# typesense/typesense

Measured on NVIDIA B200. Metric: queries/sec, higher is better.
Workload: dtype u32+f32

## Files before the change

### include/tsgpu.h

```cpp
#ifndef TSGPU_H
#define TSGPU_H
#include <stdint.h>
#include <stddef.h>

#ifdef __cplusplus
extern "C" {
#endif

typedef int tsgpu_status;
enum {
    TSGPU_OK = 0,
    TSGPU_ERR_NO_DEVICE = 1,
    TSGPU_ERR_INVALID = 2,
    TSGPU_ERR_CUDA = 3,
    TSGPU_ERR_CAPACITY = 4
};

#define TSGPU_NO_LIST 0xFFFFFFFFu
#define TSGPU_MAX_FIELDS 8
#define TSGPU_MAX_TOKENS 16
#define TSGPU_MAX_TOPK 1024

typedef struct tsgpu_index tsgpu_index;

// ... 189 lines not shown
typedef struct { uint32_t value_id, count, doc_id, array_pos; } tsgpu_facet_count;
tsgpu_status tsgpu_index_load_facet(tsgpu_index* idx, const tsgpu_facet* f, uint32_t* out_facet);
tsgpu_status tsgpu_facet_counts(tsgpu_index* idx, uint32_t facet, const uint32_t* result_ids, size_t n, uint32_t sample_mod,
                                uint32_t top_n, tsgpu_facet_count* out, uint32_t* out_n, uint32_t* out_distinct);
tsgpu_status tsgpu_facet_counts_last(tsgpu_index* idx, uint32_t facet, uint32_t top_n, tsgpu_facet_count* out, uint32_t* out_n,
                                     uint32_t* out_distinct);
tsgpu_status tsgpu_all_result_ids_last(tsgpu_index* idx, uint32_t q, uint32_t* out_ids, size_t cap, size_t* out_n);

typedef struct {
    float    ms_total;
    float    ms_kernels;
    float    ms_keyword;
    float    ms_knn;
    float    ms_fuse;
    uint64_t launches_total;
    uint64_t kw_driver_ids;
    uint64_t kw_probe_ids;
    uint64_t kw_matches;
    uint64_t knn_dist;
    uint64_t knn_expanded;
    uint64_t h2d_bytes;
    uint64_t d2h_bytes;
    float    ms_kw_search;
    float    ms_kw_merge;
    float    ms_host_plan;
    uint64_t knn_spec_hits;
    uint64_t knn_tier2_walks;
    uint64_t knn_retried;
    uint64_t h2d_total;
    uint64_t d2h_total;
    uint64_t calls_total;
    uint64_t knn_table_probes;
    uint64_t flat_tc_queries;
} tsgpu_stats;
tsgpu_status tsgpu_get_stats(tsgpu_index* idx, tsgpu_stats* out);
tsgpu_status tsgpu_debug_knn_work(tsgpu_index* idx, uint32_t* out, uint32_t cap_queries, uint32_t* out_n);

#ifdef __cplusplus
}
#endif
#endif
```

### typesense_b200/csrc/knn_kernels.cuh

```cuda
#pragma once
#include <cuda_runtime.h>
#include <stdint.h>
#include <float.h>

namespace tsv {

constexpr uint32_t kNone = 0xFFFFFFFFu;
constexpr int kKnnThreads = 128;
constexpr uint32_t kCandSmem = 256;
constexpr uint32_t kVisSmem = 2048;
constexpr uint32_t kVisSmemLimit = 1536;

struct HnswDev {
    uint32_t n_nodes, dim, M, max_level, entry_point, metric;
    const float* vectors;
    const uint32_t* labels;
    const uint8_t* levels;
    const uint32_t* links0;
    const unsigned long long* upper_off;
    const uint32_t* links_up;
    const uint32_t* deleted;
};

struct KnnParams {
    const float* queries;
    uint32_t nq, k, ef;
    const uint32_t* const* q_filter_bitmap;
    const uint32_t* const* q_excl;
    const uint32_t* q_n_excl;
    const uint8_t* q_skip;
    const uint32_t* q_order;
    uint32_t n_order;
    const uint32_t* n_order_dev;
    float* out_dist;
    uint32_t* out_labels;
    uint32_t* out_n;
    uint32_t* vis2;
    uint32_t vis2_slots;
    unsigned long long* cand;
    uint32_t cand_cap;
    uint32_t* counter;
    unsigned long long* stats;
    uint32_t* retry_n;
    uint32_t* retry_list;
    uint32_t vis_cache;
    uint32_t walk_prefetch;
    uint32_t* q_work;
};

__device__ __forceinline__ uint32_t ord_f32(float f) {
    const uint32_t u = __float_as_uint(f);
    return (u & 0x80000000u) ? ~u : (u | 0x80000000u);
}
__device__ __forceinline__ float unord_f32(uint32_t o) {
    const uint32_t u = (o & 0x80000000u) ? (o & 0x7FFFFFFFu) : ~o;
    return __uint_as_float(u);
}

template <int NCH>
struct QReg { float4 v[NCH > 0 ? NCH : 1]; };

__device__ __forceinline__ float warp_tree(float a0, float a1, float a2, float a3) {
    float t = __fadd_rn(__fadd_rn(a0, a1), __fadd_rn(a2, a3));
#pragma unroll
    for(int off = 16; off >= 1; off >>= 1) t = __fadd_rn(t, __shfl_xor_sync(0xffffffffu, t, off));
    return t;
}

template <int NCH>
__device__ __forceinline__ float dot_one(const QReg<NCH>& q, const float* __restrict__ qs, const float* __restrict__ v,
                                         uint32_t dim, uint32_t lane) {
    float a0 = 0.f, a1 = 0.f, a2 = 0.f, a3 = 0.f;
    if(NCH > 0) {
        float4 x[NCH > 0 ? NCH : 1];
#pragma unroll
        for(int s = 0; s < NCH; s++) x[s] = __ldg(reinterpret_cast<const float4*>(v + s * 128) + lane);
#pragma unroll
        for(int s = 0; s < NCH; s++) {
            a0 = __fmaf_rn(q.v[s].x, x[s].x, a0); a1 = __fmaf_rn(q.v[s].y, x[s].y, a1);
// ... 474 lines not shown
    asm volatile("mbarrier.init.shared::cta.b64 [%0], %1;" :: "r"(bar), "r"(count) : "memory");
}
__device__ __forceinline__ void mbar_expect_tx(uint32_t bar, uint32_t bytes) {
    asm volatile("mbarrier.arrive.expect_tx.shared::cta.b64 _, [%0], %1;" :: "r"(bar), "r"(bytes) : "memory");
}
__device__ __forceinline__ bool mbar_try_wait(uint32_t bar, uint32_t parity) {
    uint32_t ok;
    asm volatile("{\n\t.reg .pred p;\n\tmbarrier.try_wait.parity.shared::cta.b64 p, [%1], %2;\n\tselp.u32 %0, 1, 0, p;\n\t}"
                 : "=r"(ok) : "r"(bar), "r"(parity) : "memory");
    return ok != 0;
}
__device__ __forceinline__ void bulk_g2s(uint32_t dst, const void* src, uint32_t bytes, uint32_t bar) {
    asm volatile("cp.async.bulk.shared::cluster.global.mbarrier::complete_tx::bytes [%0], [%1], %2, [%3];"
                 :: "r"(dst), "l"(src), "r"(bytes), "r"(bar) : "memory");
}

__device__ __forceinline__ bool vis_test_and_set(uint32_t* cache, uint32_t cmask, uint32_t* table, uint32_t mask2, uint32_t node, bool* went_to_table = nullptr) {
    const uint32_t key = node + 1;
    const uint32_t h = vis_hash(node);
    uint32_t* c = cache + (h & cmask);
    if(*c == key) return false;
    if(went_to_table) *went_to_table = true;
    bool fresh = false;
    uint32_t j = (h >> 11) & mask2;
    for(;;) {
        const uint32_t old = atomicCAS(table + j, 0u, key);
        if(old == 0) { fresh = true; break; }
        if(old == key) break;
        j = (j + 1) & mask2;
    }
    *c = key;
    return fresh;
}

#ifndef TSGPU_WALK_MIN_CTAS
#define TSGPU_WALK_MIN_CTAS 5
#endif
template <int NCH, int RS>
__global__ void __launch_bounds__(32 * kWalkWarps, RS == 2 ? 2 * TSGPU_WALK_MIN_CTAS : (RS == 8 ? 2 : TSGPU_WALK_MIN_CTAS))
hnsw_walk_kernel(const __grid_constant__ HnswDev g, const __grid_constant__ KnnParams P) {
    extern __shared__ __align__(128) unsigned char smem_raw[];
    const uint32_t lane = threadIdx.x & 31, warp = threadIdx.x >> 5;
    const uint32_t slot = blockIdx.x * kWalkWarps + warp;
    const uint32_t ef = P.ef > P.k ? P.ef : P.k;
    constexpr uint32_t dim = NCH * 128, row_bytes = dim * 4;
    unsigned long long* bars = reinterpret_cast<unsigned long long*>(smem_raw);
    float* ring = reinterpret_cast<float*>(smem_raw + 128) + (size_t) warp * RS * dim;
    const uint32_t n_cache = P.vis_cache, cmask = n_cache - 1;
    uint32_t* cache = reinterpret_cast<uint32_t*>(smem_raw + 128 + (size_t) kWalkWarps * RS * row_bytes) + (size_t) warp * n_cache;
    const uint32_t bar = smem_u32(bars + warp), ring_s = smem_u32(ring);
    uint32_t parity = 0;
    if(lane == 0) mbar_init(bar, 1);
    asm volatile("fence.mbarrier_init.release.cluster;" ::: "memory");
    __syncwarp();
    uint32_t* vis2 = P.vis2 + (size_t) slot * P.vis2_slots;
    const uint32_t mask2 = P.vis2_slots - 1;
    const uint32_t limit2 = P.vis2_slots - (P.vis2_slots >> 2);
    unsigned long long* const pool0 = P.cand + (size_t) slot * P.cand_cap;
    const uint32_t pool_half = P.cand_cap >> 1;
    const uint32_t L0 = 2 * g.M + 1, LU = g.M + 1;
    const uint32_t n_tickets = P.n_order_dev ? __ldcg(P.n_order_dev) : (P.q_order ? P.n_order : P.nq);
    unsigned long long n_dist_acc = 0, n_exp_acc = 0, n_hit_acc = 0, n_t2_acc = 0, n_tab_acc = 0;
    float* const qs = nullptr;

    for(;;) {
        uint32_t qi = 0;
        if(lane == 0) qi = atomicAdd(P.counter, 1u);
        qi = __shfl_sync(0xffffffffu, qi, 0);
        if(qi >= n_tickets) break;
        if(P.q_order) qi = __ldg(P.q_order + qi);
        if(P.q_skip && P.q_skip[qi]) { if(lane == 0) P.out_n[qi] = 0; continue; }
        const float* qv = P.queries + (size_t) qi * dim;
        QReg<NCH> q;
#pragma unroll
        for(int s = 0; s < NCH; s++) q.v[s] = __ldg(reinterpret_cast<const float4*>(qv + s * 128) + lane);
        const uint32_t* fbm = P.q_filter_bitmap ? P.q_filter_bitmap[qi] : nullptr;
        const uint32_t* excl = P.q_excl ? P.q_excl[qi] : nullptr;
        const uint32_t n_excl = P.q_n_excl ? P.q_n_excl[qi] : 0;
        if(g.n_nodes == 0 || g.entry_point == kNone) { if(lane == 0) P.out_n[qi] = 0; continue; }
        for(uint32_t i = lane; i < n_cache; i += 32) cache[i] = 0;
        const unsigned long long exp0 = n_exp_acc, dist0 = n_dist_acc;

        uint32_t cur = g.entry_point;
        float curdist = 1.0f - dot_one<NCH>(q, qs, g.vectors + (size_t) cur * dim, dim, lane);
        n_dist_acc++;
        for(int level = (int) g.max_level; level > 0; level--) {
            bool changed = true;
            while(changed) {
                changed = false;
                const uint32_t* rec = g.links_up + (g.upper_off[cur] + (unsigned long long) (level - 1)) * LU;
                const uint32_t size = __ldg(rec);
                const uint32_t nb = (lane < size) ? __ldg(rec + 1 + lane) : kNone;
                for(uint32_t i = 0; i < size; i += 2) {
                    const uint32_t c0 = __shfl_sync(0xffffffffu, nb, i);
                    const uint32_t c1 = (i + 1 < size) ? __shfl_sync(0xffffffffu, nb, i + 1) : c0;
                    float d0, d1;
// ... 5 lines not shown
                }
            }
        }

        WArr<kResPerLane> R; warr_clear(R);
        WArr<kBufPerLane> B; warr_clear(B);
        uint32_t n_res = 0, n_b = 0;
        unsigned long long* nearp = pool0;
        unsigned long long* farp = pool0 + pool_half;
        uint32_t n_near = 0, n_far = 0;
        unsigned long long pv = kKeyInf;
        unsigned long long b_last = 0;
        uint32_t n_vis = 0;
        bool overflow = false;
        float lowerBound;
        __syncwarp();
        {
            const bool ok = allowed(g, fbm, excl, n_excl, cur);
            if(ok) {
                const float d = curdist;
                n_dist_acc++;
                lowerBound = d;
                warr_insert(R, res_key(d, cur), lane); n_res = 1;
                warr_insert(B, cand_key(d, cur), lane); n_b = 1; b_last = cand_key(d, cur);
            } else {
                lowerBound = FLT_MAX;
                warr_insert(B, cand_key(FLT_MAX, cur), lane); n_b = 1; b_last = cand_key(FLT_MAX, cur);
            }
            if(lane == 0) vis_test_and_set(cache, cmask, vis2, mask2, cur);
            n_vis = 1;
            __syncwarp();
        }
        uint32_t prev_spec = kNone, prev_nb2 = kNone, prev_size2 = 0;
        for(;;) {
            if(overflow) break;
            if(n_b == 0) {
                if(n_near == 0) {
                    if(n_far == 0) break;
                    unsigned long long* t = nearp; nearp = farp; farp = t;
                    n_near = n_far; n_far = 0; pv = kKeyInf;
                }
                __syncwarp();
                if(n_near > kNearMax) {
                    const uint32_t n = n_near;
                    const unsigned long long sk = nearp[(unsigned long long) lane * n >> 5];
                    uint32_t rank = 0;
#pragma unroll 8
                    for(int o = 0; o < 32; o++) rank += __shfl_sync(0xffffffffu, sk, o) < sk ? 1u : 0u;
                    uint32_t q = (32u * kNearTarget + (n >> 1)) / n;
                    q = q < 1 ? 1 : (q > 16 ? 16 : q);
                    const unsigned long long pivot = __shfl_sync(0xffffffffu, sk, __ffs(__ballot_sync(0xffffffffu, rank == q)) - 1);
                    uint32_t w = 0;
                    const uint32_t lt = (1u << lane) - 1u;
                    for(uint32_t base = 0; base < n; base += 32) {
                        const bool valid = base + lane < n;
                        const unsigned long long k = valid ? nearp[base + lane] : kKeyInf;
                        const uint32_t mb = __ballot_sync(0xffffffffu, valid && k < pivot);
                        const uint32_t ma = __ballot_sync(0xffffffffu, valid && k >= pivot);
                        if(n_far + __popc(ma) > pool_half) { overflow = true; break; }
                        if(valid) {
                            if(k < pivot) nearp[w + __popc(mb & lt)] = k;
                            else farp[n_far + __popc(ma & lt)] = k;
                        }
                        w += __popc(mb); n_far += __popc(ma);
                    }
                    if(overflow) break;
// ... 32 lines not shown
                        C = N;
                    }
                    n_near = n;
                    b_last = warr_get(B, n_b - 1);
                }
                __syncwarp();
            }
            const unsigned long long top = warr_front(B);
            const float cdist = unord_f32((uint32_t) (top >> 32));
            if(cdist > lowerBound && n_res == ef) break;
            const uint32_t cnode = ~(uint32_t) top;
            warr_pop_front(B, lane); n_b--;
            if(n_b == 0) b_last = 0;
            n_exp_acc++;

            const uint32_t* rec = g.links0 + (size_t) cnode * L0;
            const bool reuse = cnode == prev_spec;
            n_hit_acc += reuse ? 1 : 0;
            const uint32_t size = reuse ? prev_size2 : __ldg(rec);
            const uint32_t nb = reuse ? prev_nb2 : ((lane + 1 < L0) ? __ldg(rec + 1 + lane) : kNone);
            uint32_t spec = kNone, nb2 = kNone, size2 = 0;
            if(n_b) spec = ~(uint32_t) warr_front(B);
            if(spec != kNone) {
                const uint32_t* rec2 = g.links0 + (size_t) spec * L0;
                size2 = __ldg(rec2);
                nb2 = (lane + 1 < L0) ? __ldg(rec2 + 1 + lane) : kNone;
            }
            if(n_vis + 32 > limit2) { overflow = true; break; }
            uint32_t fw = 0xffffffffu, dw = 0u;
            if(lane < size && !g.labels) {
                if(fbm) fw = __ldg(fbm + (nb >> 5));
                if(g.deleted) dw = __ldg(g.deleted + (nb >> 5));
            }
            bool to_table = false;
            const bool fresh = (lane < size) && vis_test_and_set(cache, cmask, vis2, mask2, nb, &to_table);
            uint32_t mask = __ballot_sync(0xffffffffu, fresh);
            n_vis += __popc(mask);
            n_tab_acc += __popc(__ballot_sync(0xffffffffu, to_table));
            bool ok_mine = false;
            if(fresh) {
                if(g.labels) ok_mine = allowed(g, fbm, excl, n_excl, nb);
                else ok_mine = ((fw >> (nb & 31)) & 1u) && !((dw >> (nb & 31)) & 1u) && !(n_excl && is_excluded(excl, n_excl, nb));
            }
            const uint32_t ok_mask = __ballot_sync(0xffffffffu, ok_mine);
            n_dist_acc += __popc(mask);
            bool hinted = P.walk_prefetch == 0;
            auto hint_next = [&]() {
                hinted = true;
                if(spec != kNone && lane < size2) {
                    const uint32_t h2 = vis_hash(nb2);
                    if(cache[h2 & cmask] != nb2 + 1) {
                        if(P.walk_prefetch & 1u) asm volatile("prefetch.global.L2 [%0];" :: "l"(vis2 + ((h2 >> 11) & mask2)));
                        if(P.walk_prefetch & 2u) asm volatile("cp.async.bulk.prefetch.L2.global [%0], %1;" :: "l"(g.vectors + (size_t) nb2 * dim), "r"(row_bytes) : "memory");
                        if((P.walk_prefetch & 4u) && fbm && !g.labels) asm volatile("prefetch.global.L2 [%0];" :: "l"(fbm + (nb2 >> 5)));
                    }
                }
            };
            if(!mask && !hinted) hint_next();
            while(mask) {
                uint32_t grp = 0, cnt = 0;
                while(mask && cnt < (uint32_t) RS) { grp |= mask & (0u - mask); mask &= mask - 1; cnt++; }
                __syncwarp();
                asm volatile("fence.proxy.async.shared::cta;" ::: "memory");
                if(lane == 0) mbar_expect_tx(bar, cnt * row_bytes);
                __syncwarp();
                if((grp >> lane) & 1u) {
                    const uint32_t rs = __popc(grp & ((1u << lane) - 1u));
                    bulk_g2s(ring_s + rs * row_bytes, g.vectors + (size_t) nb * dim, row_bytes, bar);
                }
                if(!hinted) hint_next();
                {
                    uint32_t spins = 0;
                    while(!mbar_try_wait(bar, parity)) { if(++spins > (1u << 28)) { __trap(); } }
                    parity ^= 1u;
                }
                float dres[RS];
                {
                    float acc[RS][4];
#pragma unroll
                    for(int r = 0; r < RS; r++) { acc[r][0] = 0.f; acc[r][1] = 0.f; acc[r][2] = 0.f; acc[r][3] = 0.f; }
#pragma unroll
                    for(int sgm = 0; sgm < NCH; sgm++) {
#pragma unroll
                        for(int r = 0; r < RS; r++) {
                            if((uint32_t) r < cnt) {
                                const float4 x = reinterpret_cast<const float4*>(ring + (size_t) r * dim + sgm * 128)[lane];
                                acc[r][0] = __fmaf_rn(q.v[sgm].x, x.x, acc[r][0]); acc[r][1] = __fmaf_rn(q.v[sgm].y, x.y, acc[r][1]);
                                acc[r][2] = __fmaf_rn(q.v[sgm].z, x.z, acc[r][2]); acc[r][3] = __fmaf_rn(q.v[sgm].w, x.w, acc[r][3]);
                            }
                        }
                    }
#pragma unroll
                    for(int r = 0; r < RS; r++) dres[r] = 1.0f - warp_tree(acc[r][0], acc[r][1], acc[r][2], acc[r][3]);
                }
#pragma unroll
                for(int r = 0; r < RS; r++) {
                    if((uint32_t) r < cnt && !overflow) {
                        const int src = __ffs(grp) - 1; grp &= grp - 1;
                        const float d = dres[r];
                        const uint32_t c = __shfl_sync(0xffffffffu, nb, src);
                        const bool ok = (ok_mask >> src) & 1u;
                        if(n_res < ef || lowerBound > d) {
                            if(lane == 0) {
                                const char* lp = reinterpret_cast<const char*>(g.links0 + (size_t) c * L0);
                                asm volatile("prefetch.global.L2 [%0];" :: "l"(lp));
                                asm volatile("prefetch.global.L2 [%0];" :: "l"(lp + 128));
                            }
                            const unsigned long long ck = cand_key(d, c);
                            if(ck >= pv) { if(n_far < pool_half) { if(lane == 0) farp[n_far] = ck; n_far++; } else overflow = true; }
                            else {
                                if((n_near == 0 && n_b < kBufCap) || ck < b_last) {
                                    const unsigned long long ev = warr_insert(B, ck, lane);
                                    if(n_b < kBufCap) { n_b++; b_last = ck > b_last ? ck : b_last; }
                                    else {
                                        b_last = __shfl_sync(0xffffffffu, B.a[kBufPerLane - 1], 31);
                                        if(n_near < pool_half) { if(lane == 0) nearp[n_near] = ev; n_near++; } else overflow = true;
                                    }
                                } else { if(n_near < pool_half) { if(lane == 0) nearp[n_near] = ck; n_near++; } else overflow = true; }
                            }
                            if(ok) {
                                warr_insert(R, res_key(d, c), lane);
                                if(n_res < ef) n_res++; else warr_set_inf(R, ef, lane);
                                lowerBound = unord_f32((uint32_t) (warr_get(R, n_res - 1) >> 32));
                            }
                        }
                    }
                }
                if(overflow) break;
            }
            prev_spec = spec; prev_nb2 = nb2; prev_size2 = size2;
            __syncwarp();
        }

        if(overflow) {
            if(lane == 0) { const uint32_t r = atomicAdd(P.retry_n, 1u); P.retry_list[r] = qi; P.out_n[qi] = 0; }
        } else {
            const uint32_t n = n_res < P.k ? n_res : P.k;
            if(lane == 0) P.out_n[qi] = n;
#pragma unroll
            for(int i = 0; i < kResPerLane; i++) {
                const uint32_t e = lane * kResPerLane + i;
                if(e < n) {
                    const unsigned long long t = R.a[i];
                    const uint32_t node = (uint32_t) t;
                    P.out_dist[(size_t) qi * P.k + e] = unord_f32((uint32_t) (t >> 32));
                    P.out_labels[(size_t) qi * P.k + e] = g.labels ? g.labels[node] : node;
                }
            }
        }
        if(lane == 0 && P.q_work) { P.q_work[2 * qi] = (uint32_t) (n_exp_acc - exp0); P.q_work[2 * qi + 1] = (uint32_t) (n_dist_acc - dist0); }
        __syncwarp();
        {
            if(n_vis > kVisSmemLimit) n_t2_acc++;
            uint4* z = reinterpret_cast<uint4*>(vis2);
            for(uint32_t i = lane; i < (P.vis2_slots >> 2); i += 32) z[i] = make_uint4(0, 0, 0, 0);
        }
        __syncwarp();
    }
    if(lane == 0) { atomicAdd(P.stats + 0, n_dist_acc); atomicAdd(P.stats + 1, n_exp_acc); atomicAdd(P.stats + 2, n_hit_acc); atomicAdd(P.stats + 3, n_t2_acc); atomicAdd(P.stats + 5, n_tab_acc); }
}

struct FlatParams {
    const float* queries;
    const uint32_t* ids;
    const unsigned long long* q_off;
    uint32_t nq;
    float* out_dist;
    unsigned long long* stats;
    const uint8_t* q_skip;
};

template <int NCH>
__global__ void __launch_bounds__(256)
flat_distance_kernel(const __grid_constant__ HnswDev g, const __grid_constant__ FlatParams P, unsigned long long total) {
    extern __shared__ __align__(16) unsigned char smem_raw[];
    const uint32_t lane = threadIdx.x & 31, warp = threadIdx.x >> 5;
    const uint32_t dim = g.dim, dim_pad = (dim + 3) & ~3u;
    float* qs = reinterpret_cast<float*>(smem_raw) + (size_t) warp * dim_pad;
    const unsigned long long wid = (unsigned long long) blockIdx.x * (blockDim.x >> 5) + warp;
    const unsigned long long nw = (unsigned long long) gridDim.x * (blockDim.x >> 5);
    uint32_t cur_q = kNone;
    QReg<NCH> q;
    for(unsigned long long i = wid; i < total; i += nw) {
        uint32_t lo = 0, hi = P.nq;
        while(lo + 1 < hi) { const uint32_t mid = (lo + hi) >> 1; if(P.q_off[mid] <= i) lo = mid; else hi = mid; }
        if(P.q_skip && P.q_skip[lo]) continue;
        if(lo != cur_q) {
            cur_q = lo;
            const float* qv = P.queries + (size_t) cur_q * dim;
            if(NCH > 0) {
#pragma unroll
                for(int s = 0; s < NCH; s++) q.v[s] = __ldg(reinterpret_cast<const float4*>(qv + s * 128) + lane);
// ... 49 lines not shown
```

### typesense_b200/csrc/tsgpu.cu

```cuda
#include <cuda_runtime.h>
#include <dlfcn.h>

#include <algorithm>
#include <cstdio>
#include <cstdlib>
#include <cstring>
#include <chrono>
#include <cmath>
#include <map>
#include <mutex>
#include <random>
#include <string>
#include <vector>

#include "../../include/tsgpu.h"
#include "fuse_kernels.cuh"
#include "knn_kernels.cuh"
#include "hnsw_build.cuh"
#include "facet_kernels.cuh"
#include "postings_pack.h"

extern "C" size_t tsgpu_flat_tc_image_bytes_(uint32_t ng, uint32_t dim, uint32_t* n_tile_out, uint32_t* n_qtiles_out);
extern "C" int tsgpu_flat_tc_supported_(uint32_t dim);
extern "C" cudaError_t tsgpu_flat_tc_run_(const float* vectors, uint32_t n_nodes, uint32_t dim, const float* queries, const uint32_t* qsel, uint32_t ng,
// ... 578 lines not shown
        cudaFuncSetAttribute(tsv::hnsw_walk_kernel<NCH == 6 ? 6 : 1, 8>, cudaFuncAttributeMaxDynamicSharedMemorySize, (int) std::max<size_t>(smem, 48 * 1024));
        tsv::hnsw_walk_kernel<NCH == 6 ? 6 : 1, 8><<<grid, 32 * tsv::kWalkWarps, smem, idx->vs>>>(idx->hnsw, P);
        return;
    }
    if(NCH == 6 && rs == 2) {
        cudaFuncSetAttribute(tsv::hnsw_walk_kernel<NCH == 6 ? 6 : 1, 2>, cudaFuncAttributeMaxDynamicSharedMemorySize, (int) std::max<size_t>(smem, 48 * 1024));
        tsv::hnsw_walk_kernel<NCH == 6 ? 6 : 1, 2><<<grid, 32 * tsv::kWalkWarps, smem, idx->vs>>>(idx->hnsw, P);
        return;
    }
    cudaFuncSetAttribute(tsv::hnsw_walk_kernel<NCH, tsv::kStageRows>, cudaFuncAttributeMaxDynamicSharedMemorySize, (int) std::max<size_t>(smem, 48 * 1024));
    tsv::hnsw_walk_kernel<NCH, tsv::kStageRows><<<grid, 32 * tsv::kWalkWarps, smem, idx->vs>>>(idx->hnsw, P);
}

tsgpu_status run_knn(tsgpu_index* idx, const float* d_queries, uint32_t nq, uint32_t k, uint32_t ef,
                     const std::vector<const uint32_t*>& q_bitmap, const std::vector<const uint32_t*>& q_excl,
                     const std::vector<uint32_t>& q_nexcl, const std::vector<uint8_t>& q_skip, const std::vector<float>& q_cost,
                     KnnDeviceOut& out) {
    cudaStream_t st = idx->vs;
    if(!idx->has_hnsw) return fail(TSGPU_ERR_INVALID, "no vector index loaded");
    if(k == 0) return fail(TSGPU_ERR_INVALID, "k must be > 0");
    const uint32_t efe = std::max(ef, k);
    if(efe > 4096) return fail(TSGPU_ERR_CAPACITY, "max(ef,k) must be <= 4096");
    const tsv::HnswDev& g = idx->hnsw;
    static const bool force_heap = getenv("TSGPU_KNN_HEAP") && atoi(getenv("TSGPU_KNN_HEAP")) == 1;
    const uint32_t dim = g.dim;
    const int nch = (dim % 128 == 0 && dim / 128 <= 8 && dim / 128 != 5 && dim / 128 != 7) ? (int) (dim / 128) : 0;
    const bool walk = !force_heap && efe <= 32 * tsv::kResPerLane && 2 * g.M <= 32 && nch > 0;
    const unsigned wpc = walk ? (unsigned) tsv::kWalkWarps : 4u;
    static const int env_rs = getenv("TSGPU_WALK_ROWS") ? atoi(getenv("TSGPU_WALK_ROWS")) : 0;
    static const int env_cache = getenv("TSGPU_WALK_CACHE") ? atoi(getenv("TSGPU_WALK_CACHE")) : 0;
    static const int env_ctas = getenv("TSGPU_WALK_CTAS") ? atoi(getenv("TSGPU_WALK_CTAS")) : 0;
    const int rs = ((env_rs == 2 || env_rs == 8) && nch == 6) ? env_rs : tsv::kStageRows;
    const uint32_t vis_cache = env_cache >= 64 ? pow2_ceil((uint32_t) env_cache) : tsv::kVisCache;
    const size_t per_warp_smem = walk ? (size_t) rs * dim * 4 + (size_t) vis_cache * 4
                                      : ((size_t) efe + 1 + tsv::kCandSmem) * 8 + (size_t) tsv::kVisSmem * 4;
    const size_t q_bytes = nch ? 0 : (size_t) 4 * ((dim + 3) & ~3u) * 4;
    const size_t smem = wpc * per_warp_smem + q_bytes + (walk ? 128 : 0);
    if(smem > 200 * 1024) return fail(TSGPU_ERR_CAPACITY, "max(ef,k) / dim too large for the per-query shared-memory heaps");
    const unsigned smem_blocks = (unsigned) std::max<size_t>(1, (size_t) (227 * 1024) / (smem + 1024));
    const unsigned max_blocks = walk ? (unsigned) idx->n_sms * std::min(smem_blocks, (unsigned) (env_ctas > 0 ? env_ctas : (rs == 2 ? 2 : 1) * TSGPU_WALK_MIN_CTAS))
                                     : (unsigned) idx->n_sms * std::min(idx->knn_blocks_per_sm, smem_blocks);
    const unsigned grid = std::max(1u, std::min(max_blocks, (nq + wpc - 1) / wpc));
    const size_t slots = (size_t) grid * wpc;
    const uint32_t vis2_slots = 1u << 16, cand_cap = std::min<uint32_t>(1u << 16, std::max<uint32_t>(1024, 2 * (g.n_nodes + 1)));
    if(slots > idx->knn_slots) {
        idx->d_knn_vis.release();
        CU(idx->d_knn_vis.reserve(slots * (size_t) vis2_slots * 4));
        CU(cudaMemsetAsync(idx->d_knn_vis.p, 0, idx->d_knn_vis.cap, st));
        idx->knn_slots = slots;
    }
    CU(idx->d_knn_cand.reserve(slots * (size_t) cand_cap * 8));
    const uint32_t big_vis = pow2_ceil(std::max<uint32_t>(1u << 17, 2 * g.n_nodes + 64)), big_cand = 2 * (g.n_nodes + 1);
    {
        const size_t need = (size_t) 16 * big_vis * 4;
        if(need > idx->d_knn_retry_vis.cap) {
            idx->d_knn_retry_vis.release();
            CU(idx->d_knn_retry_vis.reserve(need));
            CU(cudaMemsetAsync(idx->d_knn_retry_vis.p, 0, idx->d_knn_retry_vis.cap, st));
        }
        CU(idx->d_knn_retry_cand.reserve((size_t) 16 * big_cand * 8));
    }
    std::vector<uint32_t> order;
    if(!q_cost.empty()) {
        order.resize(nq);
        for(uint32_t q = 0; q < nq; q++) order[q] = q;
        std::stable_sort(order.begin(), order.end(), [&](uint32_t a, uint32_t b2) { return q_cost[a] > q_cost[b2]; });
    }
// ... 8 lines not shown
    const size_t o_misc = sg.reserve(128);
    memset(sg.host.data() + o_misc, 0, 128);
    idx->knn_tables.swap(sg.host);
    const size_t tbl_bytes = idx->knn_tables.size();
    const size_t out_bytes = (size_t) nq * k * 8 + (size_t) nq * 4;
    CU(idx->d_knn_out.reserve(tbl_bytes + out_bytes + 256));
    unsigned char* base = idx->d_knn_out.as<unsigned char>();
    CU(cudaMemcpyAsync(base, idx->knn_tables.data(), tbl_bytes, cudaMemcpyHostToDevice, st));
    idx->stats.h2d_bytes += tbl_bytes;
    unsigned char* ob = base + ((tbl_bytes + 255) & ~size_t(255));
    out.dist = reinterpret_cast<float*>(ob);
    out.labels = reinterpret_cast<uint32_t*>(ob + (size_t) nq * k * 4);
    out.n = reinterpret_cast<uint32_t*>(ob + (size_t) nq * k * 8);
    out.stride = k;
    tsv::KnnParams P{};
    P.queries = d_queries; P.nq = nq; P.k = k; P.ef = ef;
    P.q_filter_bitmap = q_bitmap.empty() ? nullptr : reinterpret_cast<const uint32_t* const*>(base + o_bm);
    P.q_excl = q_excl.empty() ? nullptr : reinterpret_cast<const uint32_t* const*>(base + o_ex);
    P.q_n_excl = q_nexcl.empty() ? nullptr : reinterpret_cast<const uint32_t*>(base + o_ne);
    P.q_skip = q_skip.empty() ? nullptr : reinterpret_cast<const uint8_t*>(base + o_sk);
    P.q_order = order.empty() ? nullptr : reinterpret_cast<const uint32_t*>(base + o_or);
    P.n_order = nq; P.n_order_dev = nullptr;
    P.out_dist = out.dist; P.out_labels = out.labels; P.out_n = out.n;
    P.vis2 = idx->d_knn_vis.as<uint32_t>(); P.vis2_slots = vis2_slots;
    P.cand = idx->d_knn_cand.as<unsigned long long>(); P.cand_cap = cand_cap;
    P.counter = reinterpret_cast<uint32_t*>(base + o_misc);
    P.stats = reinterpret_cast<unsigned long long*>(base + o_misc + 8);
    P.retry_n = reinterpret_cast<uint32_t*>(base + o_misc + 40);
    P.retry_list = reinterpret_cast<uint32_t*>(base + o_rl);
    P.q_work = reinterpret_cast<uint32_t*>(base + o_wk);
    P.vis_cache = vis_cache;
    static const int env_pf = getenv("TSGPU_WALK_PREFETCH") ? atoi(getenv("TSGPU_WALK_PREFETCH")) : 5;
    P.walk_prefetch = (uint32_t) env_pf & 7u;
    idx->knn_work_dev = P.q_work; idx->knn_work_n = nq;
    tsv::KnnParams R = P;
    R.q_order = P.retry_list; R.n_order = 0; R.n_order_dev = P.retry_n; R.q_skip = nullptr;
    R.vis2 = idx->d_knn_retry_vis.as<uint32_t>(); R.vis2_slots = big_vis;
    R.cand = idx->d_knn_retry_cand.as<unsigned long long>(); R.cand_cap = big_cand;
    R.counter = reinterpret_cast<uint32_t*>(base + o_misc + 4);
    R.retry_n = reinterpret_cast<uint32_t*>(base + o_misc + 44);
    R.retry_list = reinterpret_cast<uint32_t*>(base + o_rl + (size_t) nq * 4);
    CU(cudaEventRecord(idx->ev[3], st));
    if(walk) switch(nch) {
        case 1: launch_walk<1>(idx, P, grid, smem, rs); launch_walk<1>(idx, R, 4, smem, rs); break;
        case 2: launch_walk<2>(idx, P, grid, smem, rs); launch_walk<2>(idx, R, 4, smem, rs); break;
        case 3: launch_walk<3>(idx, P, grid, smem, rs); launch_walk<3>(idx, R, 4, smem, rs); break;
        case 4: launch_walk<4>(idx, P, grid, smem, rs); launch_walk<4>(idx, R, 4, smem, rs); break;
        case 6: launch_walk<6>(idx, P, grid, smem, rs); launch_walk<6>(idx, R, 4, smem, rs); break;
        case 8: launch_walk<8>(idx, P, grid, smem, rs); launch_walk<8>(idx, R, 4, smem, rs); break;
        default: launch_walk<1>(idx, P, grid, smem, rs); launch_walk<1>(idx, R, 4, smem, rs); break;
    }
    else switch(nch) {
        case 1: launch_hnsw<1>(idx, P, grid, smem); launch_hnsw<1>(idx, R, 1, smem); break;
        case 2: launch_hnsw<2>(idx, P, grid, smem); launch_hnsw<2>(idx, R, 1, smem); break;
        case 3: launch_hnsw<3>(idx, P, grid, smem); launch_hnsw<3>(idx, R, 1, smem); break;
        case 4: launch_hnsw<4>(idx, P, grid, smem); launch_hnsw<4>(idx, R, 1, smem); break;
        case 6: launch_hnsw<6>(idx, P, grid, smem); launch_hnsw<6>(idx, R, 1, smem); break;
        case 8: launch_hnsw<8>(idx, P, grid, smem); launch_hnsw<8>(idx, R, 1, smem); break;
        default: launch_hnsw<0>(idx, P, grid, smem); launch_hnsw<0>(idx, R, 1, smem); break;
    }
    idx->stats.launches_total += 2;
    CU(cudaGetLastError());
    CU(cudaEventRecord(idx->ev[4], st));
    idx->knn_misc_dev = base + o_misc;
    return TSGPU_OK;
}

tsgpu_status finish_knn(tsgpu_index* idx) {
    if(!idx->knn_misc_dev) return TSGPU_OK;
    unsigned long long hst[6];
    CU(cudaMemcpy(hst, idx->knn_misc_dev + 8, 48, cudaMemcpyDeviceToHost));
    idx->stats.knn_table_probes += hst[5];
    idx->knn_misc_dev = nullptr;
    idx->stats.knn_dist += hst[0]; idx->stats.knn_expanded += hst[1]; idx->stats.knn_spec_hits += hst[2];
    idx->stats.knn_tier2_walks += hst[3];
    idx->stats.knn_retried += (uint32_t) hst[4];
    return TSGPU_OK;
}

int flat_tc_min_group() {
    static const int v = [] {
        if(const char* e = getenv("TSGPU_FLAT_TC")) if(atoi(e) == 0) return 0;
        if(const char* e = getenv("TSGPU_FLAT_TC_MIN")) return std::max(1, atoi(e));
        return 8;
    }();
    return v;
}

bool flat_tc_forced() { static const bool v = [] { const char* e = getenv("TSGPU_FLAT_TC"); return e && atoi(e) == 1; }(); return v; }

template <int NCH>
void launch_flat(tsgpu_index* idx, const tsv::FlatParams& P, unsigned long long total, unsigned grid, size_t smem) {
    tsv::flat_distance_kernel<NCH><<<grid, 256, smem, idx->vs>>>(idx->hnsw, P, total);
}

tsgpu_status run_flat(tsgpu_index* idx, const tsv::FlatParams& P, unsigned long long total) {
    if(total == 0) return TSGPU_OK;
    const uint32_t dim = idx->hnsw.dim;
    const int nch = (dim % 128 == 0) ? (int) (dim / 128) : 0;
    const unsigned grid = (unsigned) std::min<unsigned long long>((total + 7) / 8, (unsigned long long) idx->n_sms * 8);
    const size_t q_bytes = (size_t) 8 * ((dim + 3) & ~3u) * 4;
    switch(nch) {
        case 1: launch_flat<1>(idx, P, total, grid, 0); break;
        case 2: launch_flat<2>(idx, P, total, grid, 0); break;
        case 3: launch_flat<3>(idx, P, total, grid, 0); break;
// ... 1158 lines not shown
```

### typesense_b200/structs.py

```python
from __future__ import annotations

import ctypes as C
from dataclasses import dataclass, field
from typing import List, Optional, Sequence

import numpy as np

NO_LIST = 0xFFFFFFFF
MAX_FIELDS = 8
MAX_TOKENS = 16

SORT_NONE, SORT_TEXT_MATCH, SORT_SEQ_ID, SORT_NUMERIC, SORT_VECTOR_DISTANCE = 0, 1, 2, 3, 4
MATCH_MAX_SCORE, MATCH_MAX_WEIGHT, MATCH_SUM_SCORE = 0, 1, 2
FLAG_PRIORITIZE_EXACT_MATCH, FLAG_PRIORITIZE_TOKEN_POSITION, FLAG_PRIORITIZE_NUM_MATCHING_FIELDS = 1, 2, 4
FLAG_RERANK_HYBRID_MATCHES, FLAG_KEEP_ALL_IDS = 0x40, 0x80
CFLAG_SYNONYM, CFLAG_DEMOTE_SYNONYM = 1, 2

u8p, u16p, u32p, u64p = (C.POINTER(C.c_uint8), C.POINTER(C.c_uint16), C.POINTER(C.c_uint32), C.POINTER(C.c_uint64))
i8p, i32p, i64p, f32p = (C.POINTER(C.c_int8), C.POINTER(C.c_int32), C.POINTER(C.c_int64), C.POINTER(C.c_float))

KV_DTYPE = np.dtype([
    ("key", "<u8"), ("distinct_key", "<u8"), ("scores", "<i8", (3,)), ("text_match_score", "<i8"),
    ("vector_distance", "<f4"), ("match_score_index", "i1"), ("pad0", "u1"), ("query_index", "<u2"),
])
# ... 14 lines not shown
        ("q_flags", u8p), ("q_match_type", u8p), ("q_num_query_tokens", u8p), ("q_field_weight", u8p),
        ("c_tok_off", u32p), ("c_total_cost", u32p), ("c_n_required", u8p), ("c_flags", u8p),
        ("c_syn_orig_num_tokens", i32p), ("c_orig_num_tokens", i32p),
        ("t_list", u32p),
        ("filter_off", u64p), ("filter_ids", u32p),
    ]


class HnswStruct(C.Structure):
    _fields_ = [("n_nodes", C.c_uint32), ("dim", C.c_uint32), ("M", C.c_uint32), ("max_level", C.c_uint32),
                ("entry_point", C.c_uint32), ("metric", C.c_uint32), ("vectors", f32p), ("labels", u32p),
                ("levels", u8p), ("links0", u32p), ("upper_off", u64p), ("links_up", u32p)]


class VecParamsStruct(C.Structure):
    _fields_ = [("k", C.c_uint32), ("ef", C.c_uint32), ("flat_search_cutoff", C.c_uint32),
                ("distance_threshold", C.c_float), ("alpha", C.c_float), ("fetch_size", C.c_uint32), ("flags", C.c_uint32)]


class ArtStruct(C.Structure):
    _fields_ = [("n_nodes", C.c_uint32), ("n_children", C.c_uint32), ("n_leaves", C.c_uint32), ("root", C.c_int32),
                ("node_first_child", C.c_void_p), ("node_n_children", C.c_void_p), ("node_partial_len", C.c_void_p), ("node_partial", C.c_void_p),
                ("child_byte", C.c_void_p), ("child_ref", C.c_void_p), ("leaf_key_off", C.c_void_p), ("leaf_keys", C.c_void_p),
                ("node_rank", C.c_void_p), ("leaf_rank", C.c_void_p)]


class StatsStruct(C.Structure):
    _fields_ = [("ms_total", C.c_float), ("ms_kernels", C.c_float), ("ms_keyword", C.c_float), ("ms_knn", C.c_float),
                ("ms_fuse", C.c_float), ("launches_total", C.c_uint64), ("kw_driver_ids", C.c_uint64),
                ("kw_probe_ids", C.c_uint64), ("kw_matches", C.c_uint64), ("knn_dist", C.c_uint64),
                ("knn_expanded", C.c_uint64), ("h2d_bytes", C.c_uint64), ("d2h_bytes", C.c_uint64),
                ("ms_kw_search", C.c_float), ("ms_kw_merge", C.c_float), ("ms_host_plan", C.c_float), ("knn_spec_hits", C.c_uint64),
                ("knn_tier2_walks", C.c_uint64), ("knn_retried", C.c_uint64), ("h2d_total", C.c_uint64), ("d2h_total", C.c_uint64),
                ("calls_total", C.c_uint64), ("knn_table_probes", C.c_uint64), ("flat_tc_queries", C.c_uint64)]


def _ptr(a: Optional[np.ndarray], typ):
    if a is None:
        return C.cast(None, typ)
    assert a.flags["C_CONTIGUOUS"]
    return a.ctypes.data_as(typ)


@dataclass
class FlatField:
    list_off: np.ndarray
    ids: np.ndarray
    pos_off: np.ndarray
    positions: np.ndarray
    is_array: bool = False

    @property
    def n_lists(self) -> int:
        return len(self.list_off) - 1

    def df(self, l: int) -> int:
        return int(self.list_off[l + 1] - self.list_off[l])

    def struct(self) -> FieldStruct:
        s = FieldStruct()
        s.n_lists = self.n_lists
        s.is_array = 1 if self.is_array else 0
        s.list_off = _ptr(self.list_off, u64p)
        s.ids = _ptr(self.ids, u32p)
        s.pos_off = _ptr(self.pos_off, u64p)
        s.positions = _ptr(self.positions, u32p)
        return s
# ... 195 lines not shown
```

Baseline: 147,800.

## Pipeline speculative next-node vector fetches into second smem ring in HNSW walk

Adds a second per-warp shared-memory ring and mbarrier. While the current node's neighbours are being scored, the kernel issues bulk async loads for the speculated next node's unvisited neighbour vectors and probes the visited table for them ahead of time. When the speculation hits, their distances are computed from the prefetched ring, so the memory wait overlaps with the current node's work. This doubles ring shared memory per warp and lowers launch-bounds CTA targets, which reduces occupancy and adds register pressure. Mis-speculation also wastes bandwidth, and the deferred visited commit makes the logic more complex.

```diff
diff --git a/include/tsgpu.h b/include/tsgpu.h
--- a/include/tsgpu.h
+++ b/include/tsgpu.h
@@ -245,6 +245,7 @@
     uint64_t calls_total;
     uint64_t knn_table_probes;
     uint64_t flat_tc_queries;
+    uint64_t knn_rows_ahead;
 } tsgpu_stats;
 tsgpu_status tsgpu_get_stats(tsgpu_index* idx, tsgpu_stats* out);
 tsgpu_status tsgpu_debug_knn_work(tsgpu_index* idx, uint32_t* out, uint32_t cap_queries, uint32_t* out_n);
diff --git a/typesense_b200/csrc/knn_kernels.cuh b/typesense_b200/csrc/knn_kernels.cuh
--- a/typesense_b200/csrc/knn_kernels.cuh
+++ b/typesense_b200/csrc/knn_kernels.cuh
@@ -45,6 +45,7 @@
     uint32_t* retry_list;
     uint32_t vis_cache;
     uint32_t walk_prefetch;
+    uint32_t walk_pipe;
     uint32_t* q_work;
 };
 
@@ -585,25 +586,41 @@
     *c = key;
     return fresh;
 }
+__device__ __forceinline__ bool vis_commit(uint32_t* cache, uint32_t cmask, uint32_t* table, uint32_t mask2, uint32_t node, uint32_t j) {
+    const uint32_t key = node + 1;
+    bool fresh = false;
+    for(;;) {
+        const uint32_t old = atomicCAS(table + j, 0u, key);
+        if(old == 0) { fresh = true; break; }
+        if(old == key) break;
+        j = (j + 1) & mask2;
+    }
+    cache[vis_hash(node) & cmask] = key;
+    return fresh;
+}
 
 #ifndef TSGPU_WALK_MIN_CTAS
 #define TSGPU_WALK_MIN_CTAS 5
 #endif
+#define TSGPU_WALK_REG_CTAS(RS) ((RS) == 2 ? 6 : ((RS) == 8 ? 2 : 4))
 template <int NCH, int RS>
-__global__ void __launch_bounds__(32 * kWalkWarps, RS == 2 ? 2 * TSGPU_WALK_MIN_CTAS : (RS == 8 ? 2 : TSGPU_WALK_MIN_CTAS))
+__global__ void __launch_bounds__(32 * kWalkWarps, TSGPU_WALK_REG_CTAS(RS))
 hnsw_walk_kernel(const __grid_constant__ HnswDev g, const __grid_constant__ KnnParams P) {
     extern __shared__ __align__(128) unsigned char smem_raw[];
     const uint32_t lane = threadIdx.x & 31, warp = threadIdx.x >> 5;
     const uint32_t slot = blockIdx.x * kWalkWarps + warp;
     const uint32_t ef = P.ef > P.k ? P.ef : P.k;
     constexpr uint32_t dim = NCH * 128, row_bytes = dim * 4;
+    const bool pipe = P.walk_pipe != 0;
     unsigned long long* bars = reinterpret_cast<unsigned long long*>(smem_raw);
     float* ring = reinterpret_cast<float*>(smem_raw + 128) + (size_t) warp * RS * dim;
+    float* sring = reinterpret_cast<float*>(smem_raw + 128) + (size_t) (kWalkWarps + warp) * RS * dim;
     const uint32_t n_cache = P.vis_cache, cmask = n_cache - 1;
-    uint32_t* cache = reinterpret_cast<uint32_t*>(smem_raw + 128 + (size_t) kWalkWarps * RS * row_bytes) + (size_t) warp * n_cache;
+    uint32_t* cache = reinterpret_cast<uint32_t*>(smem_raw + 128 + (size_t) (pipe ? 2 : 1) * kWalkWarps * RS * row_bytes) + (size_t) warp * n_cache;
     const uint32_t bar = smem_u32(bars + warp), ring_s = smem_u32(ring);
-    uint32_t parity = 0;
-    if(lane == 0) mbar_init(bar, 1);
+    const uint32_t sbar = smem_u32(bars + kWalkWarps + warp), sring_s = smem_u32(sring);
+    uint32_t parity = 0, sparity = 0;
+    if(lane == 0) { mbar_init(bar, 1); mbar_init(sbar, 1); }
     asm volatile("fence.mbarrier_init.release.cluster;" ::: "memory");
     __syncwarp();
     uint32_t* vis2 = P.vis2 + (size_t) slot * P.vis2_slots;
@@ -613,8 +630,31 @@
     const uint32_t pool_half = P.cand_cap >> 1;
     const uint32_t L0 = 2 * g.M + 1, LU = g.M + 1;
     const uint32_t n_tickets = P.n_order_dev ? __ldcg(P.n_order_dev) : (P.q_order ? P.n_order : P.nq);
-    unsigned long long n_dist_acc = 0, n_exp_acc = 0, n_hit_acc = 0, n_t2_acc = 0, n_tab_acc = 0;
+    unsigned long long n_dist_acc = 0, n_exp_acc = 0, n_hit_acc = 0, n_t2_acc = 0, n_tab_acc = 0, n_ahead_acc = 0;
     float* const qs = nullptr;
+    auto wait_bar = [&](uint32_t b, uint32_t& ph) {
+        uint32_t spins = 0;
+        while(!mbar_try_wait(b, ph)) { if(++spins > (1u << 28)) { __trap(); } }
+        ph ^= 1u;
+    };
+    auto ring_dots = [&](const QReg<NCH>& q, const float* rg, uint32_t cnt, float (&dres)[RS]) {
+        float acc[RS][4];
+#pragma unroll
+        for(int r = 0; r < RS; r++) { acc[r][0] = 0.f; acc[r][1] = 0.f; acc[r][2] = 0.f; acc[r][3] = 0.f; }
+#pragma unroll
+        for(int sgm = 0; sgm < NCH; sgm++) {
+#pragma unroll
+            for(int r = 0; r < RS; r++) {
+                if((uint32_t) r < cnt) {
+                    const float4 x = reinterpret_cast<const float4*>(rg + (size_t) r * dim + sgm * 128)[lane];
+                    acc[r][0] = __fmaf_rn(q.v[sgm].x, x.x, acc[r][0]); acc[r][1] = __fmaf_rn(q.v[sgm].y, x.y, acc[r][1]);
+                    acc[r][2] = __fmaf_rn(q.v[sgm].z, x.z, acc[r][2]); acc[r][3] = __fmaf_rn(q.v[sgm].w, x.w, acc[r][3]);
+                }
+            }
+        }
+#pragma unroll
+        for(int r = 0; r < RS; r++) dres[r] = 1.0f - warp_tree(acc[r][0], acc[r][1], acc[r][2], acc[r][3]);
+    };
 
     for(;;) {
         uint32_t qi = 0;
@@ -686,6 +726,8 @@
             __syncwarp();
         }
         uint32_t prev_spec = kNone, prev_nb2 = kNone, prev_size2 = 0;
+        uint32_t sp_node = kNone, sp_rows = 0, sp_st = 0, sp_slot = 0;
+        bool sp_wait = false;
         for(;;) {
             if(overflow) break;
             if(n_b == 0) {
@@ -784,8 +826,19 @@
                 if(fbm) fw = __ldg(fbm + (nb >> 5));
                 if(g.deleted) dw = __ldg(g.deleted + (nb >> 5));
             }
-            bool to_table = false;
-            const bool fresh = (lane < size) && vis_test_and_set(cache, cmask, vis2, mask2, nb, &to_table);
+            const bool ahead = pipe && cnode == sp_node;
+            bool to_table = false, fresh = false;
+            if(ahead) {
+                if(lane < size && sp_st != 0) {
+                    to_table = true;
+                    if(sp_st == 2) fresh = vis_commit(cache, cmask, vis2, mask2, nb, sp_slot);
+                    else cache[vis_hash(nb) & cmask] = nb + 1;
+                }
+            } else fresh = (lane < size) && vis_test_and_set(cache, cmask, vis2, mask2, nb, &to_table);
+            const uint32_t rows_in = ahead ? sp_rows : 0u;
+            float sres[RS];
+            if(sp_wait) { wait_bar(sbar, sparity); sp_wait = false; }
+            if(rows_in) ring_dots(q, sring, __popc(rows_in), sres);
             uint32_t mask = __ballot_sync(0xffffffffu, fresh);
             n_vis += __popc(mask);
             n_tab_acc += __popc(__ballot_sync(0xffffffffu, to_table));
@@ -796,6 +849,9 @@
             }
             const uint32_t ok_mask = __ballot_sync(0xffffffffu, ok_mine);
             n_dist_acc += __popc(mask);
+            const uint32_t sgrp = mask & rows_in;
+            mask &= ~sgrp;
+            n_ahead_acc += sgrp ? 1 : 0;
             bool hinted = P.walk_prefetch == 0;
             auto hint_next = [&]() {
                 hinted = true;
@@ -808,9 +864,10 @@
                     }
                 }
             };
-            if(!mask && !hinted) hint_next();
-            while(mask) {
-                uint32_t grp = 0, cnt = 0;
+            uint32_t grp = 0, cnt = 0;
+            bool issued = false;
+            auto issue_rows = [&]() {
+                grp = 0; cnt = 0;
                 while(mask && cnt < (uint32_t) RS) { grp |= mask & (0u - mask); mask &= mask - 1; cnt++; }
                 __syncwarp();
                 asm volatile("fence.proxy.async.shared::cta;" ::: "memory");
@@ -820,69 +877,103 @@
                     const uint32_t rs = __popc(grp & ((1u << lane) - 1u));
                     bulk_g2s(ring_s + rs * row_bytes, g.vectors + (size_t) nb * dim, row_bytes, bar);
                 }
-                if(!hinted) hint_next();
-                {
-                    uint32_t spins = 0;
-                    while(!mbar_try_wait(bar, parity)) { if(++spins > (1u << 28)) { __trap(); } }
-                    parity ^= 1u;
-                }
+                issued = true;
+            };
+            if(mask) issue_rows();
+            if(!hinted) hint_next();
+            auto admit = [&](int src, float d) {
+                const uint32_t c = __shfl_sync(0xffffffffu, nb, src);
+                const bool ok = (ok_mask >> src) & 1u;
+                if(n_res < ef || lowerBound > d) {
+                    if(lane == 0) {
+                        const char* lp = reinterpret_cast<const char*>(g.links0 + (size_t) c * L0);
+                        asm volatile("prefetch.global.L2 [%0];" :: "l"(lp));
+                        asm volatile("prefetch.global.L2 [%0];" :: "l"(lp + 128));
+                    }
+                    const unsigned long long ck = cand_key(d, c);
+                    if(ck >= pv) { if(n_far < pool_half) { if(lane == 0) farp[n_far] = ck; n_far++; } else overflow = true; }
+                    else {
+                        if((n_near == 0 && n_b < kBufCap) || ck < b_last) {
+                            const unsigned long long ev = warr_insert(B, ck, lane);
+                            if(n_b < kBufCap) { n_b++; b_last = ck > b_last ? ck : b_last; }
+                            else {
+                                b_last = __shfl_sync(0xffffffffu, B.a[kBufPerLane - 1], 31);
+                                if(n_near < pool_half) { if(lane == 0) nearp[n_near] = ev; n_near++; } else overflow = true;
+                            }
+                        } else { if(n_near < pool_half) { if(lane == 0) nearp[n_near] = ck; n_near++; } else overflow = true; }
+                    }
+                    if(ok) {
+                        warr_insert(R, res_key(d, c), lane);
+                        if(n_res < ef) n_res++; else warr_set_inf(R, ef, lane);
+                        lowerBound = unord_f32((uint32_t) (warr_get(R, n_res - 1) >> 32));
+                    }
+                }
+            };
+            uint32_t p_key = 0, p_j = 0, p_v = 0;
+            bool p_tab = false;
+            if(pipe && spec != kNone) {
+                __syncwarp();
+                if(lane < size2) {
+                    const uint32_t h2 = vis_hash(nb2);
+                    p_key = nb2 + 1;
+                    if(cache[h2 & cmask] != p_key) { p_tab = true; p_j = (h2 >> 11) & mask2; p_v = __ldcg(vis2 + p_j); }
+                }
+            }
+            if(sgrp) {
+                uint32_t sg = sgrp;
+#pragma unroll
+                for(int r = 0; r < RS; r++) {
+                    if(sg && !overflow) {
+                        const int src = __ffs(sg) - 1; sg &= sg - 1;
+                        const uint32_t slot = __popc(rows_in & ((1u << src) - 1u));
+                        float d = sres[0];
+#pragma unroll
+                        for(int s = 1; s < RS; s++) if(slot == (uint32_t) s) d = sres[s];
+                        admit(src, d);
+                    }
+                }
+            }
+            if(pipe) {
+                sp_node = spec; sp_rows = 0; sp_st = 0;
+                if(p_tab) {
+                    for(;;) {
+                        if(p_v == 0) { sp_st = 2; sp_slot = p_j; break; }
+                        if(p_v == p_key) { sp_st = 1; break; }
+                        p_j = (p_j + 1) & mask2;
+                        p_v = __ldcg(vis2 + p_j);
+                    }
+                }
+                uint32_t absent = __ballot_sync(0xffffffffu, sp_st == 2), cnt2 = 0;
+                while(absent && cnt2 < (uint32_t) RS) { sp_rows |= absent & (0u - absent); absent &= absent - 1; cnt2++; }
+                if(cnt2) {
+                    __syncwarp();
+                    asm volatile("fence.proxy.async.shared::cta;" ::: "memory");
+                    if(lane == 0) mbar_expect_tx(sbar, cnt2 * row_bytes);
+                    __syncwarp();
+                    if((sp_rows >> lane) & 1u)
+                        bulk_g2s(sring_s + __popc(sp_rows & ((1u << lane) - 1u)) * row_bytes, g.vectors + (size_t) nb2 * dim, row_bytes, sbar);
+                    sp_wait = true;
+                }
+            }
+            while(issued) {
+                wait_bar(bar, parity);
                 float dres[RS];
-                {
-                    float acc[RS][4];
-#pragma unroll
-                    for(int r = 0; r < RS; r++) { acc[r][0] = 0.f; acc[r][1] = 0.f; acc[r][2] = 0.f; acc[r][3] = 0.f; }
-#pragma unroll
-                    for(int sgm = 0; sgm < NCH; sgm++) {
-#pragma unroll
-                        for(int r = 0; r < RS; r++) {
-                            if((uint32_t) r < cnt) {
-                                const float4 x = reinterpret_cast<const float4*>(ring + (size_t) r * dim + sgm * 128)[lane];
-                                acc[r][0] = __fmaf_rn(q.v[sgm].x, x.x, acc[r][0]); acc[r][1] = __fmaf_rn(q.v[sgm].y, x.y, acc[r][1]);
-                                acc[r][2] = __fmaf_rn(q.v[sgm].z, x.z, acc[r][2]); acc[r][3] = __fmaf_rn(q.v[sgm].w, x.w, acc[r][3]);
-                            }
-                        }
-                    }
-#pragma unroll
-                    for(int r = 0; r < RS; r++) dres[r] = 1.0f - warp_tree(acc[r][0], acc[r][1], acc[r][2], acc[r][3]);
-                }
+                ring_dots(q, ring, cnt, dres);
 #pragma unroll
                 for(int r = 0; r < RS; r++) {
                     if((uint32_t) r < cnt && !overflow) {
                         const int src = __ffs(grp) - 1; grp &= grp - 1;
-                        const float d = dres[r];
-                        const uint32_t c = __shfl_sync(0xffffffffu, nb, src);
-                        const bool ok = (ok_mask >> src) & 1u;
-                        if(n_res < ef || lowerBound > d) {
-                            if(lane == 0) {
-                                const char* lp = reinterpret_cast<const char*>(g.links0 + (size_t) c * L0);
-                                asm volatile("prefetch.global.L2 [%0];" :: "l"(lp));
-                                asm volatile("prefetch.global.L2 [%0];" :: "l"(lp + 128));
-                            }
-                            const unsigned long long ck = cand_key(d, c);
-                            if(ck >= pv) { if(n_far < pool_half) { if(lane == 0) farp[n_far] = ck; n_far++; } else overflow = true; }
-                            else {
-                                if((n_near == 0 && n_b < kBufCap) || ck < b_last) {
-                                    const unsigned long long ev = warr_insert(B, ck, lane);
-                                    if(n_b < kBufCap) { n_b++; b_last = ck > b_last ? ck : b_last; }
-                                    else {
-                                        b_last = __shfl_sync(0xffffffffu, B.a[kBufPerLane - 1], 31);
-                                        if(n_near < pool_half) { if(lane == 0) nearp[n_near] = ev; n_near++; } else overflow = true;
-                                    }
-                                } else { if(n_near < pool_half) { if(lane == 0) nearp[n_near] = ck; n_near++; } else overflow = true; }
-                            }
-                            if(ok) {
-                                warr_insert(R, res_key(d, c), lane);
-                                if(n_res < ef) n_res++; else warr_set_inf(R, ef, lane);
-                                lowerBound = unord_f32((uint32_t) (warr_get(R, n_res - 1) >> 32));
-                            }
-                        }
+                        admit(src, dres[r]);
                     }
                 }
+                issued = false;
                 if(overflow) break;
+                if(mask) issue_rows();
             }
             prev_spec = spec; prev_nb2 = nb2; prev_size2 = size2;
             __syncwarp();
         }
+        if(sp_wait) wait_bar(sbar, sparity);
 
         if(overflow) {
             if(lane == 0) { const uint32_t r = atomicAdd(P.retry_n, 1u); P.retry_list[r] = qi; P.out_n[qi] = 0; }
@@ -909,7 +1000,7 @@
         }
         __syncwarp();
     }
-    if(lane == 0) { atomicAdd(P.stats + 0, n_dist_acc); atomicAdd(P.stats + 1, n_exp_acc); atomicAdd(P.stats + 2, n_hit_acc); atomicAdd(P.stats + 3, n_t2_acc); atomicAdd(P.stats + 5, n_tab_acc); }
+    if(lane == 0) { atomicAdd(P.stats + 0, n_dist_acc); atomicAdd(P.stats + 1, n_exp_acc); atomicAdd(P.stats + 2, n_hit_acc); atomicAdd(P.stats + 3, n_t2_acc); atomicAdd(P.stats + 5, n_tab_acc); atomicAdd(P.stats + 6, n_ahead_acc); }
 }
 
 struct FlatParams {
diff --git a/typesense_b200/csrc/tsgpu.cu b/typesense_b200/csrc/tsgpu.cu
--- a/typesense_b200/csrc/tsgpu.cu
+++ b/typesense_b200/csrc/tsgpu.cu
@@ -634,7 +634,9 @@
     static const int env_ctas = getenv("TSGPU_WALK_CTAS") ? atoi(getenv("TSGPU_WALK_CTAS")) : 0;
     const int rs = ((env_rs == 2 || env_rs == 8) && nch == 6) ? env_rs : tsv::kStageRows;
     const uint32_t vis_cache = env_cache >= 64 ? pow2_ceil((uint32_t) env_cache) : tsv::kVisCache;
-    const size_t per_warp_smem = walk ? (size_t) rs * dim * 4 + (size_t) vis_cache * 4
+    const char* env_pipe = getenv("TSGPU_WALK_PIPE");
+    const bool walk_pipe = !(env_pipe && atoi(env_pipe) == 0);
+    const size_t per_warp_smem = walk ? (size_t) (walk_pipe ? 2 : 1) * rs * dim * 4 + (size_t) vis_cache * 4
                                       : ((size_t) efe + 1 + tsv::kCandSmem) * 8 + (size_t) tsv::kVisSmem * 4;
     const size_t q_bytes = nch ? 0 : (size_t) 4 * ((dim + 3) & ~3u) * 4;
     const size_t smem = wpc * per_warp_smem + q_bytes + (walk ? 128 : 0);
@@ -709,6 +711,7 @@
     P.vis_cache = vis_cache;
     static const int env_pf = getenv("TSGPU_WALK_PREFETCH") ? atoi(getenv("TSGPU_WALK_PREFETCH")) : 5;
     P.walk_prefetch = (uint32_t) env_pf & 7u;
+    P.walk_pipe = walk_pipe ? 1u : 0u;
     idx->knn_work_dev = P.q_work; idx->knn_work_n = nq;
     tsv::KnnParams R = P;
     R.q_order = P.retry_list; R.n_order = 0; R.n_order_dev = P.retry_n; R.q_skip = nullptr;
@@ -745,9 +748,10 @@
 
 tsgpu_status finish_knn(tsgpu_index* idx) {
     if(!idx->knn_misc_dev) return TSGPU_OK;
-    unsigned long long hst[6];
-    CU(cudaMemcpy(hst, idx->knn_misc_dev + 8, 48, cudaMemcpyDeviceToHost));
+    unsigned long long hst[7];
+    CU(cudaMemcpy(hst, idx->knn_misc_dev + 8, 56, cudaMemcpyDeviceToHost));
     idx->stats.knn_table_probes += hst[5];
+    idx->stats.knn_rows_ahead += hst[6];
     idx->knn_misc_dev = nullptr;
     idx->stats.knn_dist += hst[0]; idx->stats.knn_expanded += hst[1]; idx->stats.knn_spec_hits += hst[2];
     idx->stats.knn_tier2_walks += hst[3];
diff --git a/typesense_b200/structs.py b/typesense_b200/structs.py
--- a/typesense_b200/structs.py
+++ b/typesense_b200/structs.py
@@ -70,7 +70,8 @@
                 ("knn_expanded", C.c_uint64), ("h2d_bytes", C.c_uint64), ("d2h_bytes", C.c_uint64),
                 ("ms_kw_search", C.c_float), ("ms_kw_merge", C.c_float), ("ms_host_plan", C.c_float), ("knn_spec_hits", C.c_uint64),
                 ("knn_tier2_walks", C.c_uint64), ("knn_retried", C.c_uint64), ("h2d_total", C.c_uint64), ("d2h_total", C.c_uint64),
-                ("calls_total", C.c_uint64), ("knn_table_probes", C.c_uint64), ("flat_tc_queries", C.c_uint64)]
+                ("calls_total", C.c_uint64), ("knn_table_probes", C.c_uint64), ("flat_tc_queries", C.c_uint64),
+                ("knn_rows_ahead", C.c_uint64)]
 
 
 def _ptr(a: Optional[np.ndarray], typ):
```

Result: slower. 125,800, median of 6 (-14.9%).
